# burn-research/OpenMEASURE

Hardware: AMD Instinct MI355X
Metric: SPR fit+reconstruct throughput (GB/s snapshot matrix) (higher is better)
Workload: dtype f64

## Files before the change

### include/spr_hip.h

```cpp
#ifndef SPR_HIP_H
#define SPR_HIP_H

#include <stddef.h>
#include <stdint.h>

#ifdef __cplusplus
extern "C" {
#endif

#define SPR_OK 0
#define SPR_E_INVALID (-1)
#define SPR_E_UNSUPPORTED (-2)
#define SPR_E_HIP (-3)
#define SPR_E_WORKSPACE (-4)

#define SPR_MAX_M 256
#define SPR_MAX_M_WIDE 512
#define SPR_MAX_R 128
#define SPR_MAX_R_STREAM 256
#define SPR_MAX_R_WIDE 1024

#define SPR_ABI_VERSION 5
int spr_abi_version(void);
const char *spr_last_error(void);
// ... 474 lines not shown
int spr_project_stream_norms_x32(const float *d_X, int64_t n_rows, int32_t m, int64_t ldx, int64_t row0,
                                 int64_t n_points, int32_t n_features, int32_t center, const double *d_inv_scale,
                                 const double *d_rowmean, const double *d_W, int32_t r, float *d_Ur, int64_t ldu,
                                 double *d_rownorm2, void *d_workspace, size_t workspace_bytes, void *stream);
int spr_project_stream_norms_x32_f64out(const float *d_X, int64_t n_rows, int32_t m, int64_t ldx, int64_t row0,
                                        int64_t n_points, int32_t n_features, int32_t center,
                                        const double *d_inv_scale, const double *d_rowmean, const double *d_W,
                                        int32_t r, double *d_Ur, int64_t ldu, double *d_rownorm2, void *d_workspace,
                                        size_t workspace_bytes, void *stream);
int spr_stats_gram_shifted_x32(const float *d_X, int64_t n_rows, int32_t m, int64_t ldx, int64_t row0,
                               int64_t n_points, int32_t n_features, const double *d_shift, double *d_rowsum,
                               void *d_workspace, size_t workspace_bytes, void *stream);
int spr_scale_rows_x32(const float *d_X, int64_t n_rows, int32_t m, int64_t ldx, int64_t row0,
                       int64_t n_points, int32_t n_features, const double *d_rowmean,
                       const double *d_inv_scale, double *d_X0, int64_t ldo, void *stream);
int spr_feature_minmax_x32(const float *d_X, int64_t n_rows, int32_t m, int64_t ldx, int64_t row0,
                           int64_t n_points, int32_t n_features, double *d_minmax,
                           void *d_workspace, size_t workspace_bytes, void *stream);
int spr_colsums_x32(const float *d_X, int64_t n_rows, int32_t m, int64_t ldx, int64_t row0,
                    int64_t n_points, int32_t n_features, const double *d_rowmean, double *d_out,
                    void *d_workspace, size_t workspace_bytes, void *stream);
int spr_feature_digit_hist_x32(const float *d_X, int64_t n_rows, int32_t m, int64_t ldx, int64_t row0,
                               int64_t n_points, int32_t n_features, const uint64_t *d_prefix, int32_t shift,
                               int32_t bits, int32_t two_targets, uint64_t *d_hist, void *stream);
int spr_synth_f32(float *d_X, int64_t n_rows, int32_t ncols, int64_t ldx, int64_t row0,
                  int64_t n_points, int32_t col0, const double *d_R, int32_t k, int32_t ldr,
                  double eps, uint64_t seed, void *stream);
int spr_reconstruct_u32(const float *d_Ur, int64_t n_rows, int32_t r, int64_t ldu, int64_t row0,
                        int64_t n_points, int32_t n_features, const double *d_rowmean,
                        const double *d_scale, const double *d_rowscale, const double *d_A, int32_t n_p,
                        double *d_Xrec, int64_t ldo, void *stream);
int spr_mask_rows_u32(float *d_Ur, int64_t n_rows, int32_t r, int64_t ldu,
                      const uint8_t *d_mask, void *stream);
int spr_qr_init_u32(const float *d_Ur, int64_t n_rows, int32_t r, int64_t ldu,
                    int64_t row0, double *d_nrm, double *d_rec, double *d_tau,
                    void *d_workspace, size_t workspace_bytes, void *stream);
int spr_qr_init_norms_u32(const float *d_Ur, int64_t n_rows, int32_t r, int64_t ldu, int64_t row0,
                          const double *d_nrm0, double *d_nrm, double *d_rec, double *d_tau,
                          void *d_workspace, size_t workspace_bytes, void *stream);
int spr_qr_epoch_sweep_u32(const float *d_Ur, int64_t n_rows, int32_t r, int64_t ldu, int64_t row0,
                           const double *d_Q, const int64_t *d_piv, int32_t j_e, int32_t j, int32_t j_mark,
                           double *d_nrm_e, double *d_nrm, const int32_t *d_pool, const int32_t *d_pool_n,
                           int64_t pool_n_host, double tau_floor, double *d_rec, double *d_tau,
                           void *d_workspace, size_t workspace_bytes, void *stream);
int spr_qr_refresh_u32(const float *d_Ur, int64_t n_rows, int32_t r, int64_t ldu, int64_t row0,
                       const double *d_Q, const int64_t *d_piv, int32_t j0, int32_t nq,
                       double *d_nrm, double *d_rec, double *d_tau,
                       void *d_workspace, size_t workspace_bytes, void *stream);
int spr_measure_csr_u32(const int64_t *d_indptr, const int64_t *d_indices, const double *d_vals,
                        int32_t s, const float *d_Ur, int64_t n_rows, int32_t r, int64_t ldu,
                        int64_t row0, const double *d_rowmean, const double *d_scale, int64_t n_points,
                        int32_t n_features, double *d_Theta, double *d_cnt, double *d_scl, void *stream);

#ifdef __cplusplus
}
#endif
#endif
```

### openmeasure_amd/_lib.py

```python
from __future__ import annotations

import ctypes as C
import os

_HERE = os.path.dirname(os.path.abspath(__file__))
LIB_PATH = os.environ.get('SPR_HIP_LIBRARY') or os.path.join(_HERE, 'libspr_hip.so')

SPR_ABI_VERSION = 5
SPR_MAX_M = 256
SPR_MAX_M_WIDE = 512
SPR_MAX_R = 128
SPR_MAX_R_STREAM = 256
SPR_MAX_R_WIDE = 1024
SPR_GP_MAX_M = 800
SPR_GP_MAX_D = 8
SPR_CK_MAX_P = SPR_GP_MAX_D + 2

_i32, _i64, _u64, _sz = C.c_int32, C.c_int64, C.c_uint64, C.c_size_t
_p = C.c_void_p
_dbl = C.c_double

PROTOTYPES = {
    'spr_abi_version': (C.c_int, []),
    'spr_last_error': (C.c_char_p, []),
    'spr_device_cus': (C.c_int, [C.POINTER(C.c_int)]),
    'spr_upload_bytes': (C.c_int, [_p, _p, _i64, _p]),
    'spr_download_bytes': (C.c_int, [_p, _p, _i64, _p, _u64, _p]),
    'spr_host_tridiag_vectors': (C.c_int, [_p, _p, _i32, _p, _i32, _p, _i32]),
    'spr_host_eig_top': (C.c_int, [_p, _i32, _i32, _p, _p, _p, _p, _p]),
    'spr_host_svd_top': (C.c_int, [_p, _i32, _i32, _p, _p, _p, _p, _p]),
    'spr_stats_gram_workspace': (_sz, [_i32, _i32]),
    'spr_stats_gram_f64': (C.c_int, [_p, _i64, _i32, _i64, _i64, _i64, _i32, _i32, _p, _p, _sz, _p]),
    'spr_stats_gram_finalize_f64': (C.c_int, [_i64, _i32, _i64, _i64, _i32, _p, _sz, _p, _p, _i32, _i32, _p]),
    'spr_stats_gram_shifted_f64': (C.c_int, [_p, _i64, _i32, _i64, _i64, _i64, _i32, _p, _p, _p, _sz, _p]),
    'spr_gram_shift_finish_f64': (C.c_int, [_p, _p, _i64, _i32, _i32, _p, _i32, _p]),
    'spr_rowstats_workspace': (_sz, [_i32]),
    'spr_rowstats_f64': (C.c_int, [_p, _i64, _i32, _i64, _i64, _i64, _i32, _p, _p, _p, _sz, _p]),
    'spr_gram_cross_workspace': (_sz, [_i32, _i32]),
    'spr_gram_cross_f64': (C.c_int, [_p, _i64, _i32, _i64, _i64, _i64, _i32, _i32, _p, _p, _p, _sz, _p]),
    'spr_gram_cross_pair_f64': (C.c_int, [_p, _i64, _i32, _i32, _i32, _i32, _i64, _i64, _i64, _i32, _i32, _p, _p, _p, _sz, _p]),
    'spr_rowmean_stats_f64': (C.c_int, [_p, _i64, _i64, _i64, _i32, _p, _p, _sz, _p]),
    'spr_spectrum_max_m': (_i32, []),
    'spr_spectrum_f64': (C.c_int, [_p, _p, _i32, _i32, _i32, _i32, _i32, _p, _p, _p, _p, _p, _p, _p, _p, _p, _p, _p]),
    'spr_gram_combine_f64': (C.c_int, [_p, _p, _i32, _i32, _i32, _i32, _p, _p, _p, _p, _p]),
    'spr_project_f64': (C.c_int, [_p, _i64, _i32, _i64, _i64, _i64, _i32, _i32, _p, _p, _p, _i32, _p, _i64, _i32, _p]),
    'spr_project_norms_supported': (_i32, [_i32, _i32, _i64, _i64, _p, _i32]),
    'spr_project_norms_f64': (C.c_int, [_p, _i64, _i32, _i64, _i64, _i64, _i32, _i32, _p, _p, _p, _i32, _p, _i64, _p, _p]),
    'spr_project_stream_norms_f64': (C.c_int, [_p, _i64, _i32, _i64, _i64, _i64, _i32, _i32, _p, _p, _p, _i32, _p, _i64, _p, _p, _sz, _p]),
    'spr_project_field_max': (_i32, []),
    'spr_project_field_f64': (C.c_int, [_p, _i64, _i32, _i64, _i64, _i64, _i32, _p, _p, _p, _i32, _p, _i64, _p, _p, _p, _i32, _p, _i64, _p]),
    'spr_project_stream_workspace': (_sz, [_i32, _i32, _i32]),
    'spr_project_stream_f64': (C.c_int, [_p, _i64, _i32, _i64, _i64, _i64, _i32, _i32, _p, _p, _p, _i32, _p, _i64, _p, _sz, _p]),
    'spr_scale_rows_f64': (C.c_int, [_p, _i64, _i32, _i64, _i64, _i64, _i32, _p, _p, _p, _i64, _p]),
    'spr_unscale_f64': (C.c_int, [_p, _i64, _i64, _i64, _i32, _p, _p, _p, _p, _p]),
    'spr_feature_minmax_workspace': (_sz, [_i32]),
    'spr_feature_minmax_f64': (C.c_int, [_p, _i64, _i32, _i64, _i64, _i64, _i32, _p, _p, _sz, _p]),
    'spr_feature_digit_hist_f64': (C.c_int, [_p, _i64, _i32, _i64, _i64, _i64, _i32, _p, _i32, _i32, _i32, _p, _p]),
    'spr_colsums_workspace': (_sz, [_i32, _i32]),
    'spr_colsums_f64': (C.c_int, [_p, _i64, _i32, _i64, _i64, _i64, _i32, _p, _p, _p, _sz, _p]),
    'spr_fill_feature_f64': (C.c_int, [_p, _i64, _i64, _i64, _i32, _p, _p]),
    'spr_reconstruct_f64': (C.c_int, [_p, _i64, _i32, _i64, _i64, _i64, _i32, _p, _p, _p, _p, _i32, _p, _i64, _p]),
    'spr_bound_sweep_workspace': (_sz, [_i32, _i32]),
    'spr_bound_sweep_f64': (C.c_int, [_p, _i64, _i32, _i64, _i64, _i64, _i32, _p, _p, _p, _p, _p, _i32, _dbl, _i32, _p, _p, _sz, _p]),
    'spr_bound_sweep_batch_workspace': (_sz, [_i32, _i32]),
    'spr_bound_sweep_batch_f64': (C.c_int, [_p, _i64, _i32, _i64, _i64, _i64, _i32, _p, _p, _p, _p, _p, _i32, _dbl, _i32, _p, _p, _sz, _p]),
    'spr_encode_workspace': (_sz, [_i32, _i32, _i32]),
    'spr_encode_f64': (C.c_int, [_p, _i64, _i32, _i64, _p, _i32, _i64, _i64, _i64, _i32, _p, _p, _p, _p, _sz, _p]),
    'spr_field_error_workspace': (_sz, [_i32, _i32]),
    'spr_field_error_f64': (C.c_int, [_p, _i64, _i32, _i64, _i64, _i64, _i32, _p, _p, _p, _i32, _p, _i64, _p, _p, _sz, _p]),
    'spr_gappy_normal_workspace': (_sz, [_i32, _i32, _i32]),
    'spr_gappy_normal_f64': (C.c_int, [_p, _i64, _i32, _i64, _p, _i32, _i64, _i64, _i64, _i32, _p, _p, _p, _i64, _p, _p, _p, _p, _sz, _p]),
    'spr_subspace_residual_workspace': (_sz, [_i32, _i32, _i32]),
    'spr_subspace_residual_f64': (C.c_int, [_p, _i64, _i32, _i64, _p, _i32, _i64, _i64, _i64, _i32, _p, _p, _p, _p, _p, _p, _p, _sz, _p]),
    'spr_basis_update_f64': (C.c_int, [_p, _i64, _i32, _i64, _p, _i32, _i64, _i64, _i64, _i32, _p, _p, _p, _p, _i32, _p, _i64, _p]),
    'spr_gappy_fill_workspace': (_sz, []),
    'spr_gappy_rowfill_f64': (C.c_int, [_p, _i64, _i32, _i64, _i64, _p, _i64, _p, _p, _sz, _p]),
    'spr_gappy_fill_f64': (C.c_int, [_p, _i64, _i32, _i64, _p, _i32, _i64, _i64, _i64, _i32, _p, _p, _p, _p, _i64, _p, _p, _sz, _p]),
    'spr_field_std_diag_f64': (C.c_int, [_p, _i64, _i32, _i64, _i64, _i64, _i32, _p, _p, _p, _i32, _p, _i64, _p]),
    'spr_field_std_factor_f64': (C.c_int, [_p, _i64, _i32, _i64, _i64, _i64, _i32, _p, _p, _p, _i32, _i32, _p, _i64, _p]),
    'spr_design_sweep_workspace': (_sz, [_i32, _i32]),
    'spr_design_sweep_f64': (C.c_int, [_p, _i64, _i32, _i64, _i64, _i64, _i32, _p, _p, _p, _i32, _p, _p, _p, _sz, _p]),
    'spr_gp_workspace': (_sz, [_i32, _i32]),
    'spr_gp_train_f64': (C.c_int, [_p, _i32, _i32, _i64, _p, _i32, _i64, _i32, _p, _dbl, _i32, _dbl, _p, _p, _p, _p, _p, _sz, _p]),
    'spr_gp_predict_f64': (C.c_int, [_p, _i32, _i32, _i64, _p, _i32, _i64, _i32, _p, _i32, _p, _p, _p, _p, _p]),
    'spr_gp_workspace_ard': (_sz, [_i32, _i32, _i32]),
    'spr_gp_train_ard_f64': (C.c_int, [_p, _i32, _i32, _i64, _p, _i32, _i64, _i32, _i32, _p, _dbl, _i32, _dbl, _p, _p, _p, _p, _p, _sz, _p]),
    'spr_gp_predict_ard_f64': (C.c_int, [_p, _i32, _i32, _i64, _p, _i32, _i64, _i32, _i32, _p, _i32, _p, _p, _p, _p, _p]),
# ... 148 lines not shown
```

### openmeasure_amd/csrc/stats_gram.hip

```cpp
#include <type_traits>

#include "rowtile.hpp"
#include "launch.hpp"

#define GRAM_MFMA(a, b, c) __builtin_amdgcn_mfma_f64_16x16x4f64((a), (b), (c), 0, 0, 0)

namespace {

template <int MT>
struct GramShape {
  static constexpr int MPAD = 16 * MT;
  static constexpr int MP = MPAD + ((MT % 2 == 0) ? 16 : 0);
  static constexpr int T = MT * (MT + 1) / 2;
  static constexpr int NU = (MT + 1) / 2;
};

template <int MT> struct GramCfg;
template <> struct GramCfg<1>  { static constexpr int NW = 8,  R = 64, KS = 8; static constexpr bool DBUF = true; static constexpr int LPRMAX = 16; };
template <> struct GramCfg<2>  { static constexpr int NW = 8,  R = 32, KS = 8; static constexpr bool DBUF = true; static constexpr int LPRMAX = 16; };
template <> struct GramCfg<3>  { static constexpr int NW = 8,  R = 64, KS = 4; static constexpr bool DBUF = true; static constexpr int LPRMAX = 16; };
template <> struct GramCfg<4>  { static constexpr int NW = 8,  R = 64, KS = 4; static constexpr bool DBUF = true; static constexpr int LPRMAX = 8; };
template <> struct GramCfg<6>  { static constexpr int NW = 12, R = 48, KS = 4; static constexpr bool DBUF = true; static constexpr int LPRMAX = 16; };
template <> struct GramCfg<8>  { static constexpr int NW = 8,  R = 32, KS = 2; static constexpr bool DBUF = true; static constexpr int LPRMAX = 16; };
template <> struct GramCfg<12> { static constexpr int NW = 12, R = 24, KS = 2; static constexpr bool DBUF = false; static constexpr int LPRMAX = 32; };
template <> struct GramCfg<16> { static constexpr int NW = 8,  R = 32, KS = 1; static constexpr bool DBUF = false; static constexpr int LPRMAX = 16; };

template <int MT> struct GramOut { static constexpr int KSO = (GramCfg<MT>::KS >= 4) ? 1 : GramCfg<MT>::KS; };

constexpr int tri_index(int mt, int ti, int tj) { return ti * mt - ti * (ti - 1) / 2 + (tj - ti); }

template <int MT>
__device__ inline void tile_coords(int idx, int &ti, int &tj) {
  ti = 0;
  while (ti < MT - 1 && idx >= MT - ti) { idx -= MT - ti; ++ti; }
  tj = ti + idx;
  if (tj > MT - 1) tj = MT - 1;
}

template <int MT, int U, int VEC, typename TX>
__device__ inline void gram_wave(const TX *__restrict__ X, int64_t ldx, int m, int center,
                                 int64_t lo, int64_t hi, int wl, int wpf, int ks, int wave, int lane,
                                 double *__restrict__ lds0, double *__restrict__ lds1,
                                 double *__restrict__ rowmean, double *__restrict__ stat_part,
                                 double *__restrict__ slab, double *__restrict__ rowsum) {
  using S = GramShape<MT>;
  using C = GramCfg<MT>;
  constexpr int R = C::R, KS = C::KS, NW = C::NW, MP = S::MP, T = S::T;
  constexpr int KROWS = R / KS, KSTEPS = KROWS / 4;
  constexpr int RA = U, RB = MT - 1 - U;
  constexpr int NA = MT - RA;
  constexpr int NB = (RB != RA) ? MT - RB : 0;
  static_assert(KROWS % 4 == 0, "k slice must be a multiple of the MFMA depth");
  using RT = RowTile<MT, R, MP, NW, C::LPRMAX, TX>;

  f64x4 accA[NA];
  f64x4 accB[NB > 0 ? NB : 1];
#pragma unroll
  for (int j = 0; j < NA; ++j) accA[j] = (f64x4){0.0, 0.0, 0.0, 0.0};
#pragma unroll
  for (int j = 0; j < NB; ++j) accB[j] = (f64x4){0.0, 0.0, 0.0, 0.0};

  RowStats st;
  st.init();
  RT tile;

  const int64_t nchunks = (hi - lo + R - 1) / R;
  int64_t c = wl;
  const double *mean_in = rowmean;
  tile.template load<VEC>(X, ldx, m, lo + c * R, hi, wave, lane, mean_in);
  tile.template center_store<true>(lds0, m, center, lo + c * R, hi, wave, lane, rowmean, &st, rowsum);
  int64_t cn = c + wpf;
  int64_t nrow0 = (cn < nchunks) ? lo + cn * R : hi;
  tile.template load<VEC>(X, ldx, m, nrow0, hi, wave, lane, mean_in);
  int buf = 0;
  const int frag = (lane >> 4) * MP + (lane & 15) + ks * KROWS * MP + RA * 16;
  while (c < nchunks) {
    double *cur = buf ? lds1 : lds0;
    double *nxt = buf ? lds0 : lds1;
    const int64_t c2 = cn + wpf;
    const int64_t n2row0 = (c2 < nchunks) ? lo + c2 * R : hi;
    __syncthreads();
    const double *p = cur + frag;
    if constexpr (C::DBUF) {
      double op[2][NA];
#pragma unroll
      for (int j = 0; j < NA; ++j) op[0][j] = p[16 * j];
#pragma unroll
      for (int k = 0; k < KSTEPS; ++k) {
        if (k + 1 < KSTEPS) {
#pragma unroll
// ... 50 lines not shown
          double *tp = red + tri_index(MT, RA, RA + j) * 256;
          tp[0] = accA[j].x; tp[64] = accA[j].y; tp[128] = accA[j].z; tp[192] = accA[j].w;
        }
#pragma unroll
        for (int j = 0; j < NB; ++j) {
          double *tp = red + tri_index(MT, RB, RB + j) * 256;
          tp[0] = accB[j].x; tp[64] = accB[j].y; tp[128] = accB[j].z; tp[192] = accB[j].w;
        }
      }
      __syncthreads();
      if (ks == s - 1) {
#pragma unroll
        for (int j = 0; j < NA; ++j) {
          const double *tp = red + tri_index(MT, RA, RA + j) * 256;
          accA[j].x += tp[0]; accA[j].y += tp[64]; accA[j].z += tp[128]; accA[j].w += tp[192];
        }
#pragma unroll
        for (int j = 0; j < NB; ++j) {
          const double *tp = red + tri_index(MT, RB, RB + j) * 256;
          accB[j].x += tp[0]; accB[j].y += tp[64]; accB[j].z += tp[128]; accB[j].w += tp[192];
        }
      }
    }
  }
  if (KSO == KS || ks == 0) {
    double *sp = slab + ((int64_t)blockIdx.x * KSO + (KSO == KS ? ks : 0)) * T * 256 + lane;
#pragma unroll
    for (int j = 0; j < NA; ++j) {
      double *tp = sp + (int64_t)tri_index(MT, RA, RA + j) * 256;
      tp[0] = accA[j].x; tp[64] = accA[j].y; tp[128] = accA[j].z; tp[192] = accA[j].w;
    }
#pragma unroll
    for (int j = 0; j < NB; ++j) {
      double *tp = sp + (int64_t)tri_index(MT, RB, RB + j) * 256;
      tp[0] = accB[j].x; tp[64] = accB[j].y; tp[128] = accB[j].z; tp[192] = accB[j].w;
    }
  }
  if ((lane % RT::LPR) == 0) {
    double *q = stat_part + ((int64_t)blockIdx.x * RT::ROWS_PER_IT + wave * RT::RPW + lane / RT::LPR) * 3;
    q[0] = st.cnt; q[1] = st.mean(); q[2] = st.m2();
  }
}

__device__ inline void chan_merge(double &n, double &mu, double &m2, double nb, double mb, double sb) {
  if (nb > 0.0) {
    const double tot = n + nb, d = mb - mu;
    mu += d * nb / tot;
    m2 += sb + d * d * n * nb / tot;
    n = tot;
  }
}

template <int MT, int U, typename TX, bool EXT, bool SUMS>
__device__ inline void gram_wave_own(const TX *__restrict__ X, int64_t ldx, int64_t lo, int64_t hi, int wl, int wpf, int ks,
                                     int wave, int lane, double *__restrict__ lds0, double *__restrict__ lds1,
                                     double *__restrict__ rowmean, double *__restrict__ slab, double *__restrict__ rowsum) {
  using S = GramShape<MT>;
  using C = GramCfg<MT>;
  constexpr int R = C::R, KS = C::KS, NW = C::NW, MP = S::MP, T = S::T;
  constexpr int KROWS = R / KS, KSTEPS = KROWS / 4;
  constexpr int RA = U, RB = MT - 1 - U;
  constexpr int NA = MT - RA;
  constexpr int NB = (RB != RA) ? MT - RB : 0;
  using RT = RowTile<MT, R, MP, NW, C::LPRMAX, TX>;

  f64x4 accA[NA];
  f64x4 accB[NB > 0 ? NB : 1];
#pragma unroll
  for (int j = 0; j < NA; ++j) accA[j] = (f64x4){0.0, 0.0, 0.0, 0.0};
#pragma unroll
  for (int j = 0; j < NB; ++j) accB[j] = (f64x4){0.0, 0.0, 0.0, 0.0};

  RT tile;
  const int64_t nchunks = (hi - lo + R - 1) / R;
  const int64_t lane_off = (int64_t)(wave * RT::RPW + lane / RT::LPR) * ldx;
  auto base_of = [&](int64_t row0) { return X + row0 * ldx; };
  int64_t c = wl;
  int64_t crow0 = lo + c * R;
#pragma unroll
  for (int it = 0; it < RT::IT; ++it) tile.template load_pass_own<EXT>(it, base_of(crow0), ldx, lane_off, hi - crow0, wave, lane, rowmean, crow0);
  if (crow0 + R <= hi) {
#pragma unroll
    for (int it = 0; it < RT::IT; ++it) tile.template center_store_own<true, EXT, SUMS>(it, lds0, crow0, hi - crow0, wave, lane, rowmean, rowsum);
  } else {
#pragma unroll
    for (int it = 0; it < RT::IT; ++it) tile.template center_store_own<false, EXT, SUMS>(it, lds0, crow0, hi - crow0, wave, lane, rowmean, rowsum);
  }
  int64_t cn = c + wpf;
  int64_t nrow0 = (cn < nchunks) ? lo + cn * R : hi;
#pragma unroll
  for (int it = 0; it < RT::IT; ++it) tile.template load_pass_own<EXT>(it, base_of(nrow0 < hi ? nrow0 : lo), ldx, lane_off, hi - nrow0, wave, lane, rowmean, nrow0 < hi ? nrow0 : lo);
  int buf = 0;
  const int frag = (lane >> 4) * MP + (lane & 15) + ks * KROWS * MP + RA * 16;
  while (c < nchunks) {
    double *cur = buf ? lds1 : lds0;
    double *nxt = buf ? lds0 : lds1;
    const int64_t c2 = cn + wpf;
    const int64_t n2row0 = (c2 < nchunks) ? lo + c2 * R : hi;
    const TX *n2base = base_of(n2row0 < hi ? n2row0 : lo);
    const bool nfull = nrow0 + R <= hi;
    __syncthreads();
    const double *p = cur + frag;
    auto stage = [&](auto full_tag, int k) {
      constexpr bool FULL = decltype(full_tag)::value;
#pragma unroll
      for (int it = 0; it < RT::IT; ++it)
        if ((it * KSTEPS) / RT::IT == k) {
          tile.template center_store_own<FULL, EXT, SUMS>(it, nxt, nrow0, hi - nrow0, wave, lane, rowmean, rowsum);
          tile.template load_pass_own<EXT>(it, n2base, ldx, lane_off, hi - n2row0, wave, lane, rowmean, n2row0 < hi ? n2row0 : lo);
        }
    };
    if constexpr (C::DBUF) {
      double op[2][NA];
#pragma unroll
      for (int j = 0; j < NA; ++j) op[0][j] = p[16 * j];
#pragma unroll
      for (int k = 0; k < KSTEPS; ++k) {
        if (k + 1 < KSTEPS) {
#pragma unroll
          for (int j = 0; j < NA; ++j) op[(k + 1) & 1][j] = p[(k + 1) * 4 * MP + 16 * j];
        }
#pragma unroll
        for (int j = 0; j < NA; ++j) accA[j] = GRAM_MFMA(op[k & 1][0], op[k & 1][j], accA[j]);
#pragma unroll
        for (int j = 0; j < NB; ++j) accB[j] = GRAM_MFMA(op[k & 1][RB - RA], op[k & 1][RB - RA + j], accB[j]);
        if (nfull) stage(std::true_type{}, k); else stage(std::false_type{}, k);
      }
    } else {
#pragma unroll
      for (int k = 0; k < KSTEPS; ++k) {
        double op[NA];
#pragma unroll
        for (int j = 0; j < NA; ++j) op[j] = p[k * 4 * MP + 16 * j];
#pragma unroll
        for (int j = 0; j < NA; ++j) accA[j] = GRAM_MFMA(op[0], op[j], accA[j]);
#pragma unroll
        for (int j = 0; j < NB; ++j) accB[j] = GRAM_MFMA(op[RB - RA], op[RB - RA + j], accB[j]);
        if (nfull) stage(std::true_type{}, k); else stage(std::false_type{}, k);
      }
    }
    buf ^= 1;
    c = cn;
    cn = c2;
    nrow0 = n2row0;
  }
  double *sp = slab + ((int64_t)blockIdx.x * KS + ks) * T * 256 + lane;
#pragma unroll
  for (int j = 0; j < NA; ++j) {
    double *tp = sp + (int64_t)tri_index(MT, RA, RA + j) * 256;
    tp[0] = accA[j].x; tp[64] = accA[j].y; tp[128] = accA[j].z; tp[192] = accA[j].w;
  }
#pragma unroll
  for (int j = 0; j < NB; ++j) {
    double *tp = sp + (int64_t)tri_index(MT, RB, RB + j) * 256;
    tp[0] = accB[j].x; tp[64] = accB[j].y; tp[128] = accB[j].z; tp[192] = accB[j].w;
  }
}

template <int MT, typename TX, bool EXT, bool SUMS>
__global__ __launch_bounds__(GramCfg<MT>::NW * 64) void stats_gram_own_kernel(
    const TX *__restrict__ X, int64_t ldx, SegPlan plan, double *__restrict__ rowmean, double *__restrict__ slab,
    double *__restrict__ rowsum) {
  using S = GramShape<MT>;
  using C = GramCfg<MT>;
  constexpr int NU = S::NU;
  __shared__ double lds[2][C::R * S::MP];
  int f, wl, wpf, base;
  int64_t lo, hi;
  if (!seg_locate(plan, blockIdx.x, f, wl, wpf, base, lo, hi)) return;
  const int lane = threadIdx.x & 63;
  const int wave = __builtin_amdgcn_readfirstlane(threadIdx.x >> 6);
  const int ks = wave / NU;
  const int unit = (NU == 8 && C::KS == 1) ? ((wave < 4) ? wave : 11 - wave) : wave % NU;
#define GRAM_UNIT(UV)                                                                                          \
  case UV:                                                                                                     \
    if constexpr (UV < NU)                                                                                     \
      gram_wave_own<MT, UV, TX, EXT, SUMS>(X, ldx, lo, hi, wl, wpf, ks, wave, lane, lds[0], lds[1], rowmean, slab, rowsum); \
    break;
  switch (unit) {
    GRAM_UNIT(0) GRAM_UNIT(1) GRAM_UNIT(2) GRAM_UNIT(3) GRAM_UNIT(4) GRAM_UNIT(5) GRAM_UNIT(6) GRAM_UNIT(7)
    default: break;
  }
#undef GRAM_UNIT
}

constexpr int RS_THREADS = 1024;
__global__ __launch_bounds__(RS_THREADS) void gram_rowmean_stats_kernel(const double *__restrict__ rowmean, SegPlan plan,
                                                                        int slots_per_wg, double *__restrict__ stat_part) {
  __shared__ double sn[RS_THREADS / 64], smu[RS_THREADS / 64], sm2[RS_THREADS / 64];
  int f, wl, wpf, base;
  int64_t lo, hi;
  if (!seg_locate(plan, blockIdx.x, f, wl, wpf, base, lo, hi)) return;
  const int lane = threadIdx.x & 63, wave = threadIdx.x >> 6;
  RowStats st;
  st.init();
  const int64_t step = (int64_t)wpf * RS_THREADS;
  int64_t row = lo + (int64_t)wl * RS_THREADS + threadIdx.x;
  for (; row + 3 * step < hi; row += 4 * step) {
    const double a = rowmean[row], b = rowmean[row + step], c = rowmean[row + 2 * step], d = rowmean[row + 3 * step];
    st.push(a, true); st.push(b, true); st.push(c, true); st.push(d, true);
  }
  for (; row < hi; row += step) st.push(rowmean[row], true);
  double n = st.cnt, mu = st.mean(), m2 = st.m2();
  for (int o = 32; o > 0; o >>= 1) {
    const double on = __shfl_down(n, o, 64), om = __shfl_down(mu, o, 64), os = __shfl_down(m2, o, 64);
    chan_merge(n, mu, m2, on, om, os);
  }
  if (lane == 0) { sn[wave] = n; smu[wave] = mu; sm2[wave] = m2; }
  __syncthreads();
  double *q = stat_part + (int64_t)blockIdx.x * slots_per_wg * 3;
  if (threadIdx.x == 0) {
    n = 0.0; mu = 0.0; m2 = 0.0;
    for (int w = 0; w < RS_THREADS / 64; ++w) chan_merge(n, mu, m2, sn[w], smu[w], sm2[w]);
    q[0] = n; q[1] = mu; q[2] = m2;
  }
  for (int e = 3 + threadIdx.x; e < slots_per_wg * 3; e += RS_THREADS) q[e] = 0.0;
}

template <int MT, int VEC, typename TX>
__global__ __launch_bounds__(GramCfg<MT>::NW * 64) void stats_gram_kernel(
    const TX *__restrict__ X, int64_t ldx, int m, int center_i, SegPlan plan,
    double *__restrict__ rowmean, double *__restrict__ stat_part, double *__restrict__ slab, double *__restrict__ rowsum) {
  using S = GramShape<MT>;
  using C = GramCfg<MT>;
  constexpr int NU = S::NU;
  static_assert(NU * C::KS == C::NW, "waves = units x k slices");
  __shared__ double lds[2][C::R * S::MP];

  int f, wl, wpf, base;
  int64_t lo, hi;
  if (!seg_locate(plan, blockIdx.x, f, wl, wpf, base, lo, hi)) return;

  const int lane = threadIdx.x & 63;
  const int wave = __builtin_amdgcn_readfirstlane(threadIdx.x >> 6);
  const int unit = wave % NU, ks = wave / NU;
#define GRAM_UNIT(UV)                                                                                        \
  case UV:                                                                                                   \
    if constexpr (UV < NU)                                                                                   \
      gram_wave<MT, UV, VEC, TX>(X, ldx, m, center_i, lo, hi, wl, wpf, ks, wave, lane, lds[0],    \
                        lds[1], rowmean, stat_part, slab, rowsum);                                           \
    break;
  switch (unit) {
    GRAM_UNIT(0) GRAM_UNIT(1) GRAM_UNIT(2) GRAM_UNIT(3) GRAM_UNIT(4) GRAM_UNIT(5) GRAM_UNIT(6) GRAM_UNIT(7)
    default: break;
  }
#undef GRAM_UNIT
}

template <int MT>
__global__ __launch_bounds__(1024) void gram_finalize_kernel(
    const double *__restrict__ slab, const double *__restrict__ stat_part, int m, SegPlan plan,
    int slots_per_wg, double *__restrict__ gram, double *__restrict__ fstats, int ldg, int origin) {
  constexpr int T = GramShape<MT>::T;
  constexpr int KS = GramOut<MT>::KSO;
  __shared__ double red[4][256];
  const int f = blockIdx.y;
  const int tile = blockIdx.x;
  int base = 0, wpf = 0;
  {
    int acc = 0;
    const int f0 = seg_first_feature(plan), f1 = seg_last_feature(plan);
    for (int ff = f0; ff <= f1; ++ff) {
      int64_t lo, hi;
      seg_range(plan, ff, lo, hi);
      const int w = seg_wgs(plan, hi - lo);
      if (ff == f) { base = acc; wpf = w; }
      acc += w;
    }
  }
  int ti, tj;
  tile_coords<MT>(tile, ti, tj);
  const int e = threadIdx.x & 255, g = threadIdx.x >> 8;
  const int np = wpf * KS;
  const double *sp = slab + ((int64_t)base * KS * T + tile) * 256 + e;
  const int64_t stride = (int64_t)T * 256;
  double s0 = 0.0, s1 = 0.0, s2 = 0.0, s3 = 0.0;
  int p = g;
  for (; p + 12 < np; p += 16) {
    s0 += sp[p * stride];
    s1 += sp[(p + 4) * stride];
    s2 += sp[(p + 8) * stride];
    s3 += sp[(p + 12) * stride];
  }
  for (; p < np; p += 4) s0 += sp[p * stride];
  red[g][e] = (s0 + s1) + (s2 + s3);
  __syncthreads();
  if (g == 0) {
    const double sum = (red[0][e] + red[1][e]) + (red[2][e] + red[3][e]);
    const int l = e & 63, reg = e >> 6;
    const int gi = ti * 16 + (l >> 4) + 4 * reg, gj = tj * 16 + (l & 15);
    if (gi < m && gj < m) {
      double *G = gram + (int64_t)f * ldg * ldg + (int64_t)origin * ldg + origin;
      G[(int64_t)gi * ldg + gj] = sum;
      if (ti != tj) G[(int64_t)gj * ldg + gi] = sum;
    }
  }
  if (tile == 0) {
    __syncthreads();
    double n = 0.0, mu = 0.0, m2 = 0.0;
    const double *q = stat_part + (int64_t)base * slots_per_wg * 3;
    const int tot_slots = wpf * slots_per_wg;
    for (int pp = threadIdx.x; pp < tot_slots; pp += 1024) chan_merge(n, mu, m2, q[3 * pp], q[3 * pp + 1], q[3 * pp + 2]);
    double *sn = &red[0][0], *smu = &red[1][0], *sm2 = &red[2][0];
    for (int o = 32; o > 0; o >>= 1) {
      const double on = __shfl_down(n, o, 64), om = __shfl_down(mu, o, 64), os = __shfl_down(m2, o, 64);
      chan_merge(n, mu, m2, on, om, os);
    }
    const int w = threadIdx.x >> 6;
    if ((threadIdx.x & 63) == 0) { sn[w] = n; smu[w] = mu; sm2[w] = m2; }
    __syncthreads();
    if (threadIdx.x == 0) {
      n = 0.0; mu = 0.0; m2 = 0.0;
      for (int ww = 0; ww < 16; ++ww) chan_merge(n, mu, m2, sn[ww], smu[ww], sm2[ww]);
      fstats[3 * f] = n; fstats[3 * f + 1] = mu; fstats[3 * f + 2] = m2;
    }
  }
}

template <int MT>
int occupancy_wgs() {
  static int cached = 0;
  if (cached) return cached;
  int per_cu = 0;
  if (hipOccupancyMaxActiveBlocksPerMultiprocessor(&per_cu, stats_gram_kernel<MT, 2, double>, GramCfg<MT>::NW * 64, 0) != hipSuccess ||
      per_cu < 1)
    per_cu = 1;
  if (per_cu > 4) per_cu = 4;
  cached = per_cu * spr_cus_or_default();
  return cached;
}

template <int MT>
SegPlan make_plan(int64_t n_rows, int64_t row0, int64_t n_points, int32_t n_features) {
  SegPlan p;
  p.row0 = row0; p.n_rows = n_rows; p.n_points = n_points; p.n_features = n_features;
  p.total_wg = occupancy_wgs<MT>();
  p.chunk_rows = GramCfg<MT>::R;
  return p;
}

template <int MT>
size_t workspace_bytes(int32_t n_features) {
  using RT = RowTile<MT, GramCfg<MT>::R, GramShape<MT>::MP, GramCfg<MT>::NW, GramCfg<MT>::LPRMAX>;
  const int64_t max_grid = (int64_t)occupancy_wgs<MT>() + n_features;
  return (size_t)max_grid * GramCfg<MT>::KS * GramShape<MT>::T * 256 * sizeof(double) +
         (size_t)max_grid * RT::ROWS_PER_IT * 3 * sizeof(double);
}

template <int MT, typename TX>
int launch(const TX *X, int64_t n_rows, int32_t m, int64_t ldx, int64_t row0, int64_t n_points,
           int32_t n_features, int center, double *rowmean, void *ws, size_t ws_bytes, hipStream_t st,
           double *rowsum = nullptr) {
  SPR_REQUIRE(ws_bytes >= workspace_bytes<MT>(n_features), SPR_E_WORKSPACE,
              "spr_stats_gram_f64: workspace %zu < %zu", ws_bytes, workspace_bytes<MT>(n_features));
  SPR_REQUIRE(!rowsum || center == 2, SPR_E_INVALID, "spr_stats_gram: row sums are an output of centre mode 2 only");
  SegPlan plan = make_plan<MT>(n_rows, row0, n_points, n_features);
  const int grid = seg_total_wgs(plan);
  const int64_t max_grid = (int64_t)occupancy_wgs<MT>() + n_features;
  SPR_REQUIRE(grid >= 1 && grid <= max_grid, SPR_E_INVALID, "spr_stats_gram_f64: bad grid %d", grid);
  double *slab = static_cast<double *>(ws);
  double *stat_part = slab + (size_t)max_grid * GramCfg<MT>::KS * GramShape<MT>::T * 256;
  const int lm = spr_load_mode(spr_pair_aligned(X, m, ldx), m, MT);
#define SG_LAUNCH(LM)                                                                                         \
  hipLaunchKernelGGL((stats_gram_kernel<MT, LM, TX>), dim3(grid), dim3(GramCfg<MT>::NW * 64), 0, st, X, ldx, (int)m, \
                     center, plan, rowmean, stat_part, slab, rowsum)
  using RTL = RowTile<MT, GramCfg<MT>::R, GramShape<MT>::MP, GramCfg<MT>::NW, GramCfg<MT>::LPRMAX, TX>;
  if (MT >= 8 && lm == 2 && (center == 1 || center == 2) && spr_rows_aligned16(X, sizeof(TX) * ldx)) {
    if constexpr (MT >= 8) {
      if (center == 1)
        hipLaunchKernelGGL((stats_gram_own_kernel<MT, TX, false, false>), dim3(grid), dim3(GramCfg<MT>::NW * 64), 0, st, X, ldx,
                           plan, rowmean, slab, rowsum);
      else if (!rowsum)
        hipLaunchKernelGGL((stats_gram_own_kernel<MT, TX, true, false>), dim3(grid), dim3(GramCfg<MT>::NW * 64), 0, st, X, ldx,
                           plan, rowmean, slab, rowsum);
      else
        hipLaunchKernelGGL((stats_gram_own_kernel<MT, TX, true, true>), dim3(grid), dim3(GramCfg<MT>::NW * 64), 0, st, X, ldx,
                           plan, rowmean, slab, rowsum);
      SPR_LAUNCH_CHECK();
      hipLaunchKernelGGL(gram_rowmean_stats_kernel, dim3(grid), dim3(RS_THREADS), 0, st, rowmean, plan, (int)RTL::ROWS_PER_IT,
                         stat_part);
      SPR_LAUNCH_CHECK();
      return SPR_OK;
    }
  }
  if (lm == 2) SG_LAUNCH(2);
  else if (lm == 1) SG_LAUNCH(1);
  else SG_LAUNCH(0);
#undef SG_LAUNCH
  SPR_LAUNCH_CHECK();
  return SPR_OK;
}

template <int MT>
int launch_finalize(int64_t n_rows, int32_t m, int64_t row0, int64_t n_points, int32_t n_features,
                    double *fstats, double *gram, int ldg, int origin, const void *ws, size_t ws_bytes,
                    hipStream_t st) {
  using RT = RowTile<MT, GramCfg<MT>::R, GramShape<MT>::MP, GramCfg<MT>::NW, GramCfg<MT>::LPRMAX>;
  SPR_REQUIRE(ws_bytes >= workspace_bytes<MT>(n_features), SPR_E_WORKSPACE,
              "spr_stats_gram_finalize_f64: workspace %zu < %zu", ws_bytes, workspace_bytes<MT>(n_features));
  SegPlan plan = make_plan<MT>(n_rows, row0, n_points, n_features);
  const int64_t max_grid = (int64_t)occupancy_wgs<MT>() + n_features;
  const double *slab = static_cast<const double *>(ws);
  const double *stat_part = slab + (size_t)max_grid * GramCfg<MT>::KS * GramShape<MT>::T * 256;
  hipLaunchKernelGGL(gram_finalize_kernel<MT>, dim3(GramShape<MT>::T, n_features), dim3(1024), 0, st, slab,
                     stat_part, (int)m, plan, (int)RT::ROWS_PER_IT, gram, fstats, ldg, origin);
  SPR_LAUNCH_CHECK();
  return SPR_OK;
}

int check_args(const char *who, const void *X, int64_t n_rows, int32_t m, int64_t ldx, int64_t row0,
               int64_t n_points, int32_t n_features) {
  SPR_REQUIRE(X != nullptr, SPR_E_INVALID, "%s: X is NULL", who);
  SPR_REQUIRE(n_rows > 0 && m > 0 && ldx >= m, SPR_E_INVALID, "%s: bad shape n_rows=%lld m=%d ldx=%lld", who,
              (long long)n_rows, m, (long long)ldx);
  SPR_REQUIRE(n_points > 0 && n_features > 0 && row0 >= 0, SPR_E_INVALID, "%s: bad feature layout", who);
  SPR_REQUIRE(row0 + n_rows <= n_points * (int64_t)n_features, SPR_E_INVALID,
              "%s: rows [%lld,%lld) exceed n_points*n_features=%lld", who, (long long)row0,
              (long long)(row0 + n_rows), (long long)(n_points * (int64_t)n_features));
  SPR_REQUIRE(m <= SPR_MAX_M, SPR_E_UNSUPPORTED, "%s: m=%d > %d not built", who, m, SPR_MAX_M);
  return SPR_OK;
}

}

#define GRAM_DISPATCH_M(mt, CALL)            \
  switch (mt) {                              \
    case 1: CALL(1); break;                  \
    case 2: CALL(2); break;                  \
    case 3: CALL(3); break;                  \
    case 4: CALL(4); break;                  \
    case 6: CALL(6); break;                  \
    case 8: CALL(8); break;                  \
    case 12: CALL(12); break;                \
    case 16: CALL(16); break;                \
    default: break;                          \
  }

extern "C" size_t spr_stats_gram_workspace(int32_t m, int32_t n_features) {
  if (m <= 0 || m > SPR_MAX_M || n_features <= 0) return 0;
  size_t out = 0;
#define WS_CALL(MTV) out = workspace_bytes<MTV>(n_features)
  GRAM_DISPATCH_M(spr_round_mt(m), WS_CALL)
#undef WS_CALL
  return out;
}

extern "C" int spr_stats_gram_f64(const double *d_X, int64_t n_rows, int32_t m, int64_t ldx, int64_t row0,
                                  int64_t n_points, int32_t n_features, int32_t center, double *d_rowmean,
                                  void *d_workspace, size_t workspace_bytes_, void *stream) {
  int rc = check_args("spr_stats_gram_f64", d_X, n_rows, m, ldx, row0, n_points, n_features);
  if (rc != SPR_OK) return rc;
  SPR_REQUIRE(d_rowmean && d_workspace, SPR_E_INVALID, "spr_stats_gram_f64: NULL output/workspace");
  rc = SPR_E_UNSUPPORTED;
#define RUN_CALL(MTV)                                                                                \
  rc = launch<MTV>(d_X, n_rows, m, ldx, row0, n_points, n_features, center, d_rowmean, d_workspace, \
                   workspace_bytes_, static_cast<hipStream_t>(stream))
  GRAM_DISPATCH_M(spr_round_mt(m), RUN_CALL)
#undef RUN_CALL
  return rc;
}

extern "C" int spr_stats_gram_x32(const float *d_X, int64_t n_rows, int32_t m, int64_t ldx, int64_t row0,
                                  int64_t n_points, int32_t n_features, int32_t center, double *d_rowmean,
                                  void *d_workspace, size_t workspace_bytes_, void *stream) {
  int rc = check_args("spr_stats_gram_x32", d_X, n_rows, m, ldx, row0, n_points, n_features);
  if (rc != SPR_OK) return rc;
  SPR_REQUIRE(d_rowmean && d_workspace, SPR_E_INVALID, "spr_stats_gram_x32: NULL output/workspace");
  rc = SPR_E_UNSUPPORTED;
#define RUN_CALL(MTV)                                                                                \
  rc = launch<MTV>(d_X, n_rows, m, ldx, row0, n_points, n_features, center, d_rowmean, d_workspace, \
                   workspace_bytes_, static_cast<hipStream_t>(stream))
  GRAM_DISPATCH_M(spr_round_mt(m), RUN_CALL)
#undef RUN_CALL
  return rc;
}

extern "C" int spr_stats_gram_shifted_f64(const double *d_X, int64_t n_rows, int32_t m, int64_t ldx, int64_t row0,
                                          int64_t n_points, int32_t n_features, const double *d_shift,
                                          double *d_rowsum, void *d_workspace, size_t workspace_bytes_, void *stream) {
  int rc = check_args("spr_stats_gram_shifted_f64", d_X, n_rows, m, ldx, row0, n_points, n_features);
  if (rc != SPR_OK) return rc;
  SPR_REQUIRE(d_shift && d_rowsum && d_workspace, SPR_E_INVALID, "spr_stats_gram_shifted_f64: NULL pointer");
  rc = SPR_E_UNSUPPORTED;
#define RUN_CALL(MTV)                                                                                                    \
  rc = launch<MTV>(d_X, n_rows, m, ldx, row0, n_points, n_features, 2, const_cast<double *>(d_shift), d_workspace,       \
                   workspace_bytes_, static_cast<hipStream_t>(stream), d_rowsum)
  GRAM_DISPATCH_M(spr_round_mt(m), RUN_CALL)
#undef RUN_CALL
  return rc;
}

extern "C" int spr_stats_gram_shifted_x32(const float *d_X, int64_t n_rows, int32_t m, int64_t ldx, int64_t row0,
                                          int64_t n_points, int32_t n_features, const double *d_shift,
                                          double *d_rowsum, void *d_workspace, size_t workspace_bytes_, void *stream) {
  int rc = check_args("spr_stats_gram_shifted_x32", d_X, n_rows, m, ldx, row0, n_points, n_features);
  if (rc != SPR_OK) return rc;
  SPR_REQUIRE(d_shift && d_rowsum && d_workspace, SPR_E_INVALID, "spr_stats_gram_shifted_x32: NULL pointer");
  rc = SPR_E_UNSUPPORTED;
#define RUN_CALL(MTV)                                                                                                    \
  rc = launch<MTV>(d_X, n_rows, m, ldx, row0, n_points, n_features, 2, const_cast<double *>(d_shift), d_workspace,       \
                   workspace_bytes_, static_cast<hipStream_t>(stream), d_rowsum)
  GRAM_DISPATCH_M(spr_round_mt(m), RUN_CALL)
#undef RUN_CALL
  return rc;
}

extern "C" int spr_stats_gram_finalize_f64(int64_t n_rows, int32_t m, int64_t row0, int64_t n_points,
                                           int32_t n_features, const void *d_workspace, size_t workspace_bytes_,
                                           double *d_fstats, double *d_gram, int32_t ldg, int32_t origin,
                                           void *stream) {
  int rc = check_args("spr_stats_gram_finalize_f64", d_workspace, n_rows, m, m, row0, n_points, n_features);
  if (rc != SPR_OK) return rc;
  SPR_REQUIRE(d_fstats && d_gram, SPR_E_INVALID, "spr_stats_gram_finalize_f64: NULL output");
  SPR_REQUIRE(origin >= 0 && ldg >= origin + m, SPR_E_INVALID, "spr_stats_gram_finalize_f64: block (%d,%d)+%d outside ldg=%d",
              origin, origin, m, ldg);
  rc = SPR_E_UNSUPPORTED;
#define FIN_CALL(MTV)                                                                                 \
  rc = launch_finalize<MTV>(n_rows, m, row0, n_points, n_features, d_fstats, d_gram, ldg, origin, d_workspace, \
                            workspace_bytes_, static_cast<hipStream_t>(stream))
  GRAM_DISPATCH_M(spr_round_mt(m), FIN_CALL)
#undef FIN_CALL
  return rc;
}
```

Baseline: 1203.

## Balance Gram own-kernel work by splitting row panels evenly across workgroups

Replaces the per-feature workgroup assignment in the owned-tile Gram kernel with a span plan. Total row panels across all features are divided evenly among workgroups, so one workgroup may process segments from several features, each written to its own slab. A device-side plan tag tells the finalize kernel which slab layout to reduce, and a host-side plan query is exposed. The goal is to remove load imbalance when the rows per feature do not map evenly onto workgroups, at the cost of extra slabs, extra syncs between segments and more index arithmetic in finalize.

```diff
diff --git a/include/spr_hip.h b/include/spr_hip.h
--- a/include/spr_hip.h
+++ b/include/spr_hip.h
@@ -550,6 +550,9 @@
                         int64_t row0, const double *d_rowmean, const double *d_scale, int64_t n_points,
                         int32_t n_features, double *d_Theta, double *d_cnt, double *d_scl, void *stream);
 
+int spr_gram_span_plan(int64_t n_rows, int64_t row0, int64_t n_points, int32_t n_features, int32_t m,
+                       int32_t *h_grid, int32_t *h_n_segments, int64_t *h_segments, int32_t capacity);
+
 #ifdef __cplusplus
 }
 #endif
diff --git a/openmeasure_amd/_lib.py b/openmeasure_amd/_lib.py
--- a/openmeasure_amd/_lib.py
+++ b/openmeasure_amd/_lib.py
@@ -33,6 +33,7 @@
     'spr_stats_gram_f64': (C.c_int, [_p, _i64, _i32, _i64, _i64, _i64, _i32, _i32, _p, _p, _sz, _p]),
     'spr_stats_gram_finalize_f64': (C.c_int, [_i64, _i32, _i64, _i64, _i32, _p, _sz, _p, _p, _i32, _i32, _p]),
     'spr_stats_gram_shifted_f64': (C.c_int, [_p, _i64, _i32, _i64, _i64, _i64, _i32, _p, _p, _p, _sz, _p]),
+    'spr_gram_span_plan': (C.c_int, [_i64, _i64, _i64, _i32, _i32, _p, _p, _p, _i32]),
     'spr_gram_shift_finish_f64': (C.c_int, [_p, _p, _i64, _i32, _i32, _p, _i32, _p]),
     'spr_rowstats_workspace': (_sz, [_i32]),
     'spr_rowstats_f64': (C.c_int, [_p, _i64, _i32, _i64, _i64, _i64, _i32, _p, _p, _p, _sz, _p]),
diff --git a/openmeasure_amd/csrc/stats_gram.hip b/openmeasure_amd/csrc/stats_gram.hip
--- a/openmeasure_amd/csrc/stats_gram.hip
+++ b/openmeasure_amd/csrc/stats_gram.hip
@@ -36,6 +36,41 @@
   tj = ti + idx;
   if (tj > MT - 1) tj = MT - 1;
 }
+
+__host__ __device__ inline int64_t span_feature_panels(const SegPlan &p, int f) {
+  int64_t lo, hi;
+  seg_range(p, f, lo, hi);
+  return (hi - lo + p.chunk_rows - 1) / p.chunk_rows;
+}
+
+__host__ __device__ inline int64_t span_total_panels(const SegPlan &p) {
+  int64_t tot = 0;
+  for (int f = seg_first_feature(p), f1 = seg_last_feature(p); f <= f1; ++f) tot += span_feature_panels(p, f);
+  return tot;
+}
+
+__host__ __device__ inline int64_t span_begin(const SegPlan &p, int64_t P, int g) { return (int64_t)g * P / p.total_wg; }
+
+__host__ __device__ inline int span_owner(const SegPlan &p, int64_t P, int64_t q) {
+  return (int)(((q + 1) * p.total_wg - 1) / P);
+}
+
+__host__ __device__ inline bool span_segment(const SegPlan &p, int f, int64_t fp0, int64_t pb, int64_t pe, int64_t &lo,
+                                             int64_t &hi) {
+  int64_t flo, fhi;
+  seg_range(p, f, flo, fhi);
+  const int64_t fpn = (fhi - flo + p.chunk_rows - 1) / p.chunk_rows;
+  const int64_t a = pb > fp0 ? pb : fp0, b = pe < fp0 + fpn ? pe : fp0 + fpn;
+  if (a >= b) return false;
+  lo = flo + (a - fp0) * p.chunk_rows;
+  hi = flo + (b - fp0) * p.chunk_rows;
+  if (hi > fhi) hi = fhi;
+  return true;
+}
+
+__host__ __device__ inline int span_slab(const SegPlan &p, int g, int f) { return g + (f - seg_first_feature(p)); }
+
+constexpr double GRAM_TAG_SEG = 0.0, GRAM_TAG_SPAN = 1.0;
 
 template <int MT, int U, int VEC, typename TX>
 __device__ inline void gram_wave(const TX *__restrict__ X, int64_t ldx, int m, int center,
@@ -192,9 +227,9 @@
 }
 
 template <int MT, int U, typename TX, bool EXT, bool SUMS>
-__device__ inline void gram_wave_own(const TX *__restrict__ X, int64_t ldx, int64_t lo, int64_t hi, int wl, int wpf, int ks,
-                                     int wave, int lane, double *__restrict__ lds0, double *__restrict__ lds1,
-                                     double *__restrict__ rowmean, double *__restrict__ slab, double *__restrict__ rowsum) {
+__device__ inline void gram_segment_own(const TX *__restrict__ X, int64_t ldx, int64_t lo, int64_t hi, int slab_idx, int ks,
+                                        int wave, int lane, double *__restrict__ lds0, double *__restrict__ lds1,
+                                        double *__restrict__ rowmean, double *__restrict__ slab, double *__restrict__ rowsum) {
   using S = GramShape<MT>;
   using C = GramCfg<MT>;
   constexpr int R = C::R, KS = C::KS, NW = C::NW, MP = S::MP, T = S::T;
@@ -215,7 +250,8 @@
   const int64_t nchunks = (hi - lo + R - 1) / R;
   const int64_t lane_off = (int64_t)(wave * RT::RPW + lane / RT::LPR) * ldx;
   auto base_of = [&](int64_t row0) { return X + row0 * ldx; };
-  int64_t c = wl;
+  constexpr int wpf = 1;
+  int64_t c = 0;
   int64_t crow0 = lo + c * R;
 #pragma unroll
   for (int it = 0; it < RT::IT; ++it) tile.template load_pass_own<EXT>(it, base_of(crow0), ldx, lane_off, hi - crow0, wave, lane, rowmean, crow0);
@@ -284,7 +320,7 @@
     cn = c2;
     nrow0 = n2row0;
   }
-  double *sp = slab + ((int64_t)blockIdx.x * KS + ks) * T * 256 + lane;
+  double *sp = slab + ((int64_t)slab_idx * KS + ks) * T * 256 + lane;
 #pragma unroll
   for (int j = 0; j < NA; ++j) {
     double *tp = sp + (int64_t)tri_index(MT, RA, RA + j) * 256;
@@ -297,17 +333,43 @@
   }
 }
 
+template <int MT, int U, typename TX, bool EXT, bool SUMS>
+__device__ inline void gram_wave_own(const TX *__restrict__ X, int64_t ldx, const SegPlan &plan, int64_t pb, int64_t pe, int ks,
+                                     int wave, int lane, double *__restrict__ lds0, double *__restrict__ lds1,
+                                     double *__restrict__ rowmean, double *__restrict__ slab, double *__restrict__ rowsum) {
+  bool first = true;
+  int64_t fp0 = 0;
+  for (int f = seg_first_feature(plan), f1 = seg_last_feature(plan); f <= f1 && fp0 < pe; ++f) {
+    int64_t lo, hi;
+    const bool has = span_segment(plan, f, fp0, pb, pe, lo, hi);
+    fp0 += span_feature_panels(plan, f);
+    if (!has) continue;
+    if (!first) __syncthreads();
+    first = false;
+    int ln = lane;
+    asm volatile("" : "+v"(ln));
+    gram_segment_own<MT, U, TX, EXT, SUMS>(X, ldx, lo, hi, span_slab(plan, (int)blockIdx.x, f), ks, wave, ln, lds0, lds1,
+                                           rowmean, slab, rowsum);
+  }
+}
+
 template <int MT, typename TX, bool EXT, bool SUMS>
 __global__ __launch_bounds__(GramCfg<MT>::NW * 64) void stats_gram_own_kernel(
     const TX *__restrict__ X, int64_t ldx, SegPlan plan, double *__restrict__ rowmean, double *__restrict__ slab,
-    double *__restrict__ rowsum) {
+    double *__restrict__ rowsum, double *__restrict__ plan_tag) {
   using S = GramShape<MT>;
   using C = GramCfg<MT>;
   constexpr int NU = S::NU;
   __shared__ double lds[2][C::R * S::MP];
-  int f, wl, wpf, base;
-  int64_t lo, hi;
-  if (!seg_locate(plan, blockIdx.x, f, wl, wpf, base, lo, hi)) return;
+  if (blockIdx.x == 0 && threadIdx.x == 0) *plan_tag = GRAM_TAG_SPAN;
+  plan.chunk_rows = C::R;
+  auto uniform = [](int64_t v) {
+    const uint32_t l = __builtin_amdgcn_readfirstlane((uint32_t)v), h = __builtin_amdgcn_readfirstlane((uint32_t)((uint64_t)v >> 32));
+    return (int64_t)(((uint64_t)h << 32) | l);
+  };
+  const int64_t P = span_total_panels(plan);
+  const int64_t pb = uniform(span_begin(plan, P, blockIdx.x)), pe = uniform(span_begin(plan, P, blockIdx.x + 1));
+  if (pb >= pe) return;
   const int lane = threadIdx.x & 63;
   const int wave = __builtin_amdgcn_readfirstlane(threadIdx.x >> 6);
   const int ks = wave / NU;
@@ -315,7 +377,7 @@
 #define GRAM_UNIT(UV)                                                                                          \
   case UV:                                                                                                     \
     if constexpr (UV < NU)                                                                                     \
-      gram_wave_own<MT, UV, TX, EXT, SUMS>(X, ldx, lo, hi, wl, wpf, ks, wave, lane, lds[0], lds[1], rowmean, slab, rowsum); \
+      gram_wave_own<MT, UV, TX, EXT, SUMS>(X, ldx, plan, pb, pe, ks, wave, lane, lds[0], lds[1], rowmean, slab, rowsum); \
     break;
   switch (unit) {
     GRAM_UNIT(0) GRAM_UNIT(1) GRAM_UNIT(2) GRAM_UNIT(3) GRAM_UNIT(4) GRAM_UNIT(5) GRAM_UNIT(6) GRAM_UNIT(7)
@@ -360,12 +422,14 @@
 template <int MT, int VEC, typename TX>
 __global__ __launch_bounds__(GramCfg<MT>::NW * 64) void stats_gram_kernel(
     const TX *__restrict__ X, int64_t ldx, int m, int center_i, SegPlan plan,
-    double *__restrict__ rowmean, double *__restrict__ stat_part, double *__restrict__ slab, double *__restrict__ rowsum) {
+    double *__restrict__ rowmean, double *__restrict__ stat_part, double *__restrict__ slab, double *__restrict__ rowsum,
+    double *__restrict__ plan_tag) {
   using S = GramShape<MT>;
   using C = GramCfg<MT>;
   constexpr int NU = S::NU;
   static_assert(NU * C::KS == C::NW, "waves = units x k slices");
   __shared__ double lds[2][C::R * S::MP];
+  if (blockIdx.x == 0 && threadIdx.x == 0) *plan_tag = GRAM_TAG_SEG;
 
   int f, wl, wpf, base;
   int64_t lo, hi;
@@ -390,10 +454,12 @@
 template <int MT>
 __global__ __launch_bounds__(1024) void gram_finalize_kernel(
     const double *__restrict__ slab, const double *__restrict__ stat_part, int m, SegPlan plan,
-    int slots_per_wg, double *__restrict__ gram, double *__restrict__ fstats, int ldg, int origin) {
+    int slots_per_wg, double *__restrict__ gram, double *__restrict__ fstats, int ldg, int origin,
+    const double *__restrict__ plan_tag) {
   constexpr int T = GramShape<MT>::T;
   constexpr int KS = GramOut<MT>::KSO;
   __shared__ double red[4][256];
+  plan.chunk_rows = GramCfg<MT>::R;
   const int f = blockIdx.y;
   const int tile = blockIdx.x;
   int base = 0, wpf = 0;
@@ -408,14 +474,38 @@
       acc += w;
     }
   }
+  int sbase = base, swgs = wpf;
+  const bool span = *plan_tag == GRAM_TAG_SPAN;
+  int64_t P = 0;
+  int gfirst = 0;
+  if (span) {
+    sbase = 0; swgs = 0;
+    int64_t fp0 = 0, fpn = 0;
+    for (int ff = seg_first_feature(plan), f1 = seg_last_feature(plan); ff <= f1; ++ff) {
+      const int64_t n = span_feature_panels(plan, ff);
+      if (ff == f) { fp0 = P; fpn = n; }
+      P += n;
+    }
+    if (fpn > 0) {
+      gfirst = span_owner(plan, P, fp0);
+      swgs = span_owner(plan, P, fp0 + fpn - 1) - gfirst + 1;
+      sbase = span_slab(plan, gfirst, f);
+    }
+  }
   int ti, tj;
   tile_coords<MT>(tile, ti, tj);
   const int e = threadIdx.x & 255, g = threadIdx.x >> 8;
-  const int np = wpf * KS;
-  const double *sp = slab + ((int64_t)base * KS * T + tile) * 256 + e;
+  const int np = swgs * KS;
+  const double *sp = slab + ((int64_t)sbase * KS * T + tile) * 256 + e;
   const int64_t stride = (int64_t)T * 256;
   double s0 = 0.0, s1 = 0.0, s2 = 0.0, s3 = 0.0;
   int p = g;
+  if (span && P < plan.total_wg) {
+    for (; p < np; p += 4) {
+      const int wg = gfirst + p / KS;
+      if (span_begin(plan, P, wg) < span_begin(plan, P, wg + 1)) s0 += sp[p * stride];
+    }
+  }
   for (; p + 12 < np; p += 16) {
     s0 += sp[p * stride];
     s1 += sp[(p + 4) * stride];
@@ -497,25 +587,28 @@
   SegPlan plan = make_plan<MT>(n_rows, row0, n_points, n_features);
   const int grid = seg_total_wgs(plan);
   const int64_t max_grid = (int64_t)occupancy_wgs<MT>() + n_features;
-  SPR_REQUIRE(grid >= 1 && grid <= max_grid, SPR_E_INVALID, "spr_stats_gram_f64: bad grid %d", grid);
+  SPR_REQUIRE(grid >= 1 && grid < max_grid, SPR_E_INVALID, "spr_stats_gram_f64: bad grid %d", grid);
   double *slab = static_cast<double *>(ws);
   double *stat_part = slab + (size_t)max_grid * GramCfg<MT>::KS * GramShape<MT>::T * 256;
+  double *plan_tag = stat_part - 1;
   const int lm = spr_load_mode(spr_pair_aligned(X, m, ldx), m, MT);
 #define SG_LAUNCH(LM)                                                                                         \
   hipLaunchKernelGGL((stats_gram_kernel<MT, LM, TX>), dim3(grid), dim3(GramCfg<MT>::NW * 64), 0, st, X, ldx, (int)m, \
-                     center, plan, rowmean, stat_part, slab, rowsum)
+                     center, plan, rowmean, stat_part, slab, rowsum, plan_tag)
   using RTL = RowTile<MT, GramCfg<MT>::R, GramShape<MT>::MP, GramCfg<MT>::NW, GramCfg<MT>::LPRMAX, TX>;
   if (MT >= 8 && lm == 2 && (center == 1 || center == 2) && spr_rows_aligned16(X, sizeof(TX) * ldx)) {
     if constexpr (MT >= 8) {
+      SPR_REQUIRE(plan.total_wg + (seg_last_feature(plan) - seg_first_feature(plan)) < max_grid, SPR_E_INVALID,
+                  "spr_stats_gram_f64: bad span plan");
       if (center == 1)
-        hipLaunchKernelGGL((stats_gram_own_kernel<MT, TX, false, false>), dim3(grid), dim3(GramCfg<MT>::NW * 64), 0, st, X, ldx,
-                           plan, rowmean, slab, rowsum);
+        hipLaunchKernelGGL((stats_gram_own_kernel<MT, TX, false, false>), dim3(plan.total_wg), dim3(GramCfg<MT>::NW * 64), 0, st, X,
+                           ldx, plan, rowmean, slab, rowsum, plan_tag);
       else if (!rowsum)
-        hipLaunchKernelGGL((stats_gram_own_kernel<MT, TX, true, false>), dim3(grid), dim3(GramCfg<MT>::NW * 64), 0, st, X, ldx,
-                           plan, rowmean, slab, rowsum);
+        hipLaunchKernelGGL((stats_gram_own_kernel<MT, TX, true, false>), dim3(plan.total_wg), dim3(GramCfg<MT>::NW * 64), 0, st, X,
+                           ldx, plan, rowmean, slab, rowsum, plan_tag);
       else
-        hipLaunchKernelGGL((stats_gram_own_kernel<MT, TX, true, true>), dim3(grid), dim3(GramCfg<MT>::NW * 64), 0, st, X, ldx,
-                           plan, rowmean, slab, rowsum);
+        hipLaunchKernelGGL((stats_gram_own_kernel<MT, TX, true, true>), dim3(plan.total_wg), dim3(GramCfg<MT>::NW * 64), 0, st, X,
+                           ldx, plan, rowmean, slab, rowsum, plan_tag);
       SPR_LAUNCH_CHECK();
       hipLaunchKernelGGL(gram_rowmean_stats_kernel, dim3(grid), dim3(RS_THREADS), 0, st, rowmean, plan, (int)RTL::ROWS_PER_IT,
                          stat_part);
@@ -543,7 +636,7 @@
   const double *slab = static_cast<const double *>(ws);
   const double *stat_part = slab + (size_t)max_grid * GramCfg<MT>::KS * GramShape<MT>::T * 256;
   hipLaunchKernelGGL(gram_finalize_kernel<MT>, dim3(GramShape<MT>::T, n_features), dim3(1024), 0, st, slab,
-                     stat_part, (int)m, plan, (int)RT::ROWS_PER_IT, gram, fstats, ldg, origin);
+                     stat_part, (int)m, plan, (int)RT::ROWS_PER_IT, gram, fstats, ldg, origin, stat_part - 1);
   SPR_LAUNCH_CHECK();
   return SPR_OK;
 }
@@ -643,6 +736,39 @@
   GRAM_DISPATCH_M(spr_round_mt(m), RUN_CALL)
 #undef RUN_CALL
   return rc;
+}
+
+extern "C" int spr_gram_span_plan(int64_t n_rows, int64_t row0, int64_t n_points, int32_t n_features, int32_t m,
+                                  int32_t *h_grid, int32_t *h_n_segments, int64_t *h_segments, int32_t capacity) {
+  int rc = check_args("spr_gram_span_plan", h_grid, n_rows, m, m, row0, n_points, n_features);
+  if (rc != SPR_OK) return rc;
+  SPR_REQUIRE(h_n_segments && capacity >= 0, SPR_E_INVALID, "spr_gram_span_plan: NULL count / negative capacity");
+  const int mt = spr_round_mt(m);
+  SPR_REQUIRE(mt >= 8, SPR_E_UNSUPPORTED, "spr_gram_span_plan: m=%d takes the per-feature plan", m);
+  SegPlan plan;
+#define PLAN_CALL(MTV) plan = make_plan<MTV>(n_rows, row0, n_points, n_features)
+  GRAM_DISPATCH_M(mt, PLAN_CALL)
+#undef PLAN_CALL
+  const int64_t P = span_total_panels(plan);
+  int32_t n_seg = 0;
+  for (int g = 0; g < plan.total_wg; ++g) {
+    const int64_t pb = span_begin(plan, P, g), pe = span_begin(plan, P, g + 1);
+    int64_t fp0 = 0;
+    for (int f = seg_first_feature(plan), f1 = seg_last_feature(plan); f <= f1 && fp0 < pe; ++f) {
+      int64_t lo, hi;
+      const bool has = span_segment(plan, f, fp0, pb, pe, lo, hi);
+      fp0 += span_feature_panels(plan, f);
+      if (!has) continue;
+      if (h_segments && n_seg < capacity) {
+        int64_t *q = h_segments + 5 * (int64_t)n_seg;
+        q[0] = g; q[1] = f; q[2] = lo; q[3] = hi; q[4] = span_slab(plan, g, f);
+      }
+      ++n_seg;
+    }
+  }
+  *h_grid = plan.total_wg;
+  *h_n_segments = n_seg;
+  return SPR_OK;
 }
 
 extern "C" int spr_stats_gram_finalize_f64(int64_t n_rows, int32_t m, int64_t row0, int64_t n_points,
```

After: 1207, median of 4. About the same (+0.4%).
